# facebookresearch/multipathnet

Hardware: NVIDIA H100
Metric: proposals/sec (higher is better)
Workload: dtype fp32 (wgmma split emulation, fp32 accumulate: 3 bf16 products per MAC, 2 fp16 products in fc6/fc7)

## Files before the change

### multipathnet_b200/csrc/gemm_tc.cu

```cuda
#include "conv_gemm.cuh"
#include "wgmma.cuh"
#include "fp8_e4m3.cuh"
#include <algorithm>
#include <stdlib.h>
#include <string.h>

namespace {

constexpr int BM = 128;
constexpr int BK = 64;
constexpr int TC_THREADS = 384;
constexpr int CONS_THREADS = 256;
constexpr int A_TILE_BYTES = BM * BK * 2;
constexpr int SMEM_BUDGET = 196608;

__host__ __device__ constexpr int a_planes(OperandScheme ops) { return (ops == OperandScheme::BF16X1 || ops == OperandScheme::FP8X1) ? 1 : 2; }
__host__ __device__ constexpr int b_planes(OperandScheme ops) { return ops == OperandScheme::BF16X3 ? 2 : 1; }
__host__ __device__ constexpr int elem_bytes(OperandScheme ops) { return ops == OperandScheme::FP8X1 ? 1 : 2; }
__host__ __device__ constexpr int a_tile_bytes(OperandScheme ops) { return BM * BK * elem_bytes(ops); }
__host__ __device__ constexpr int stage_bytes(int BN, OperandScheme ops = OperandScheme::BF16X3) {
  return a_planes(ops) * a_tile_bytes(ops) + b_planes(ops) * BN * BK * elem_bytes(ops);
}
__host__ __device__ constexpr int max_stages(OperandScheme ops) { return ops == OperandScheme::FP8X1 ? 8 : 4; }
__host__ __device__ constexpr int num_stages(int BN, OperandScheme ops = OperandScheme::BF16X3) {
  return (SMEM_BUDGET / stage_bytes(BN, ops)) > max_stages(ops) ? max_stages(ops) : (SMEM_BUDGET / stage_bytes(BN, ops));
}
__host__ __device__ constexpr int stg_ld(int BN) { return BN + 4; }
static_assert(BM * (256 + 4) * 4 <= 2 * stage_bytes(256), "staging tile must fit in the ring");

struct TcParams {
  int N, Ho, Wo, Cout;
  int kh, kw, stride, pad;
  int cblocks;
  int tn, th, tw;
  int tiles_img, tiles_h, tiles_w, tiles_n;
  const float *bias;
  const __nv_bfloat16 *res_hi, *res_lo; long long res_ld;
  __nv_bfloat16 *out_hi, *out_lo; long long out_ld;
  float *out_f32; long long out_f32_ld;
  __nv_bfloat16 *pool_hi, *pool_lo; long long pool_ld; int Hp, Wp;
  int relu;
  int splitk, kb_per_split;
  long long split_stride;
  unsigned long long *tl_min, *tl_max;
  float acc_scale;
  int out_fmt;
  unsigned *ovf;
  const int *a_exp, *b_exp; long long sample_pix;
};

__device__ __forceinline__ unsigned long long gtimer() {
  unsigned long long t; asm volatile("mov.u64 %0, %%globaltimer;" : "=l"(t)); return t;
}
__device__ __forceinline__ void tl_min_stamp(const unsigned long long *base_, int i) {
  if (base_) atomicMin(const_cast<unsigned long long *>(base_) + i, gtimer());
}
__device__ __forceinline__ void tl_max_stamp(const unsigned long long *base_, int i) {
  if (base_) atomicMax(const_cast<unsigned long long *>(base_) + i, gtimer());
}
__device__ __forceinline__ uint32_t smem_u32(const void *p) { return (uint32_t)__cvta_generic_to_shared(p); }
__device__ __forceinline__ void mbar_init(uint32_t bar, uint32_t count) {
  asm volatile("mbarrier.init.shared::cta.b64 [%0], %1;" ::"r"(bar), "r"(count) : "memory");
}
__device__ __forceinline__ void mbar_expect_tx(uint32_t bar, uint32_t bytes) {
  asm volatile("mbarrier.arrive.expect_tx.shared::cta.b64 _, [%0], %1;" ::"r"(bar), "r"(bytes) : "memory");
}
__device__ __forceinline__ void mbar_arrive(uint32_t bar) {
  asm volatile("mbarrier.arrive.shared::cta.b64 _, [%0];" ::"r"(bar) : "memory");
}
__device__ __forceinline__ void mbar_wait(uint32_t bar, uint32_t parity) {
  uint32_t done;
  uint32_t spins = 0;
  do {
    asm volatile(
        "{\n\t.reg .pred p;\n\t"
        "mbarrier.try_wait.parity.shared::cta.b64 p, [%1], %2;\n\t"
        "selp.u32 %0, 1, 0, p;\n\t}"
        : "=r"(done) : "r"(bar), "r"(parity) : "memory");
    if (!done && ++spins == (1u << 26)) __trap();
  } while (!done);
}
__device__ __forceinline__ void tma_load_4d(uint32_t dst, const CUtensorMap *tm, uint32_t bar, int c0, int c1,
                                            int c2, int c3) {
  asm volatile(
      "cp.async.bulk.tensor.4d.shared::cluster.global.mbarrier::complete_tx::bytes [%0], [%1, {%3, %4, %5, %6}], [%2];"
      ::"r"(dst), "l"(reinterpret_cast<uint64_t>(tm)), "r"(bar), "r"(c0), "r"(c1), "r"(c2), "r"(c3) : "memory");
}
__device__ __forceinline__ void tma_load_2d(uint32_t dst, const CUtensorMap *tm, uint32_t bar, int c0, int c1) {
  asm volatile(
      "cp.async.bulk.tensor.2d.shared::cluster.global.mbarrier::complete_tx::bytes [%0], [%1, {%3, %4}], [%2];"
      ::"r"(dst), "l"(reinterpret_cast<uint64_t>(tm)), "r"(bar), "r"(c0), "r"(c1) : "memory");
}
__device__ __forceinline__ void prefetch_tmap(const CUtensorMap *tm) {
  asm volatile("prefetch.tensormap [%0];" ::"l"(reinterpret_cast<uint64_t>(tm)) : "memory");
}
__device__ __forceinline__ void consumers_sync() { asm volatile("bar.sync 1, 256;" ::: "memory"); }

__device__ __forceinline__ uint64_t make_smem_desc(uint32_t saddr) {
  uint64_t d = 0;
  d |= (uint64_t)((saddr & 0x3FFFFu) >> 4);
  d |= (uint64_t)1 << 16;
  d |= (uint64_t)(1024 >> 4) << 32;
  d |= (uint64_t)1 << 62;
  return d;
}

__device__ __forceinline__ uint64_t make_smem_desc_64b(uint32_t saddr) {
  uint64_t d = 0;
  d |= (uint64_t)((saddr & 0x3FFFFu) >> 4);
  d |= (uint64_t)1 << 16;
  d |= (uint64_t)(512 >> 4) << 32;
  d |= (uint64_t)2 << 62;
  return d;
}

template <int BN, OperandScheme OPS>
__device__ __forceinline__ void mma_kblock(float (&acc)[BN / 2], uint64_t a_hi, uint64_t a_lo, uint64_t b_hi, uint64_t b_lo, bool first) {
  constexpr bool F16 = (OPS == OperandScheme::FP16X2);
#pragma unroll
  for (int k = 0; k < BK / 16; ++k) {
    const uint64_t adv = (uint64_t)((k * 16 * 2) >> 4);
    const uint32_t later = (first && k == 0) ? 0u : 1u;
    if constexpr (OPS == OperandScheme::BF16X1) {
      wgmma_nk16<BN, false>(acc, a_hi + adv, b_hi + adv, later);
    } else {
      wgmma_nk16<BN, F16>(acc, a_lo + adv, b_hi + adv, later);
      if (!F16) wgmma_nk16<BN, F16>(acc, a_hi + adv, b_lo + adv, 1u);
      wgmma_nk16<BN, F16>(acc, a_hi + adv, b_hi + adv, 1u);
    }
  }
}

template <int BN>
__device__ __forceinline__ void stage_acc(float *stg, const float (&acc)[BN / 2], int g, int t) {
  const int r0 = g * 64 + (t >> 5) * 16 + ((t & 31) >> 2), c0 = 2 * (t & 3);
#pragma unroll
  for (int j = 0; j < BN / 8; ++j) {
    *reinterpret_cast<float2 *>(stg + r0 * stg_ld(BN) + 8 * j + c0) = make_float2(acc[4 * j], acc[4 * j + 1]);
    *reinterpret_cast<float2 *>(stg + (r0 + 8) * stg_ld(BN) + 8 * j + c0) = make_float2(acc[4 * j + 2], acc[4 * j + 3]);
  }
}

template <int BN, OperandScheme OPS>
__device__ __forceinline__ void epilogue_row(const TcParams &p, const float *srow, int nt, bool row_ok, long long pix,
                                             float *out_f32, int ch_first, long long ppix) {
  const bool pool = (p.pool_hi != nullptr);
  const int tile_end = min(p.Cout, nt * BN + BN);
#pragma unroll 1
  for (int ch = ch_first; ch < BN / 32; ch += 2) {
    const int col0 = nt * BN + ch * 32;
    if (col0 >= tile_end) break;
    float v[32];
#pragma unroll
    for (int j = 0; j < 8; ++j) {
      const float4 x = *reinterpret_cast<const float4 *>(srow + ch * 32 + 4 * j);
      v[4 * j] = x.x; v[4 * j + 1] = x.y; v[4 * j + 2] = x.z; v[4 * j + 3] = x.w;
    }
    if (OPS == OperandScheme::FP16X2) {
#pragma unroll
      for (int e = 0; e < 32; ++e) v[e] *= p.acc_scale;
    }
    if (OPS == OperandScheme::FP8X1) {
      const int ea = row_ok ? __ldg(p.a_exp + pix / p.sample_pix) : 0;
#pragma unroll
      for (int e = 0; e < 32; ++e) v[e] *= mpn_fp8::pow2(-(ea + __ldg(p.b_exp + col0 + e)));
    }
    if (!(row_ok || pool)) continue;
#pragma unroll
    for (int g = 0; g < 4; ++g) {
      const int c = col0 + g * 8;
      if (c >= tile_end) break;
      float f[8];
#pragma unroll
      for (int e = 0; e < 8; ++e) f[e] = v[g * 8 + e];
      const bool full8 = (c + 8 <= tile_end);
      if (p.bias) {
        if (full8) {
          const float4 b0 = __ldg(reinterpret_cast<const float4 *>(p.bias + c));
          const float4 b1 = __ldg(reinterpret_cast<const float4 *>(p.bias + c + 4));
          f[0] += b0.x; f[1] += b0.y; f[2] += b0.z; f[3] += b0.w;
          f[4] += b1.x; f[5] += b1.y; f[6] += b1.z; f[7] += b1.w;
        } else {
          for (int e = 0; e < 8 && c + e < p.Cout; ++e) f[e] += __ldg(p.bias + c + e);
        }
      }
      if (p.res_hi && full8 && row_ok) {
        const uint4 rh = *reinterpret_cast<const uint4 *>(p.res_hi + pix * p.res_ld + c);
        const uint4 rl = *reinterpret_cast<const uint4 *>(p.res_lo + pix * p.res_ld + c);
        const uint32_t hh[4] = {rh.x, rh.y, rh.z, rh.w}, ll[4] = {rl.x, rl.y, rl.z, rl.w};
#pragma unroll
        for (int t = 0; t < 4; ++t) {
          float2 x = bf16x2_to_float2(hh[t]), y = bf16x2_to_float2(ll[t]);
          f[2 * t] += x.x + y.x; f[2 * t + 1] += x.y + y.y;
        }
      }
      if (p.relu) {
#pragma unroll
        for (int e = 0; e < 8; ++e) f[e] = fmaxf(f[e], 0.f);
      }
      if (p.out_hi && full8 && row_ok) {
        uint32_t oh[4], ol[4];
#pragma unroll
        for (int t = 0; t < 4; ++t) split_x2(p.out_fmt, f[2 * t], f[2 * t + 1], oh[t], ol[t], p.ovf);
        *reinterpret_cast<uint4 *>(p.out_hi + pix * p.out_ld + c) = make_uint4(oh[0], oh[1], oh[2], oh[3]);
        *reinterpret_cast<uint4 *>(p.out_lo + pix * p.out_ld + c) = make_uint4(ol[0], ol[1], ol[2], ol[3]);
      }
      if (pool) {
#pragma unroll
        for (int e = 0; e < 8; ++e) {
          float x = row_ok ? f[e] : -INFINITY;
          x = fmaxf(x, __shfl_xor_sync(0xffffffffu, x, 1));
          x = fmaxf(x, __shfl_xor_sync(0xffffffffu, x, 8));
          f[e] = x;
        }
        if (ppix >= 0 && full8) {
          uint32_t oh[4], ol[4];
#pragma unroll
          for (int t = 0; t < 4; ++t) split_x2(p.out_fmt, f[2 * t], f[2 * t + 1], oh[t], ol[t], p.ovf);
          *reinterpret_cast<uint4 *>(p.pool_hi + ppix * p.pool_ld + c) = make_uint4(oh[0], oh[1], oh[2], oh[3]);
          *reinterpret_cast<uint4 *>(p.pool_lo + ppix * p.pool_ld + c) = make_uint4(ol[0], ol[1], ol[2], ol[3]);
        }
      }
      if (out_f32 && row_ok) {
        float *o = out_f32 + pix * p.out_f32_ld + c;
        if (full8 && ((reinterpret_cast<uintptr_t>(o) & 15) == 0)) {
          reinterpret_cast<float4 *>(o)[0] = make_float4(f[0], f[1], f[2], f[3]);
          reinterpret_cast<float4 *>(o)[1] = make_float4(f[4], f[5], f[6], f[7]);
        } else {
          for (int e = 0; e < 8 && c + e < p.Cout; ++e) o[e] = f[e];
        }
      }
    }
  }
}

template <int BN, OperandScheme OPS = OperandScheme::BF16X3>
__global__ void __launch_bounds__(TC_THREADS, 1)
conv_gemm_tc_kernel(const __grid_constant__ CUtensorMap tmA_hi, const __grid_constant__ CUtensorMap tmA_lo,
                    const __grid_constant__ CUtensorMap tmB_hi, const __grid_constant__ CUtensorMap tmB_lo,
                    const TcParams p) {
  constexpr int S = num_stages(BN, OPS);
  constexpr int STAGE = stage_bytes(BN, OPS);
  constexpr int A_TILE = a_tile_bytes(OPS);
  constexpr int B_TILE_BYTES = BN * BK * elem_bytes(OPS);
  constexpr int B_OFF = a_planes(OPS) * A_TILE;
  static_assert(BM * stg_ld(BN) * 4 <= S * STAGE, "staging tile must fit in the ring");
  extern __shared__ uint8_t smem_raw[];
  uint8_t *smem = reinterpret_cast<uint8_t *>((reinterpret_cast<uintptr_t>(smem_raw) + 1023) & ~(uintptr_t)1023);
  uint64_t *bars = reinterpret_cast<uint64_t *>(smem + (size_t)S * STAGE);
  const uint32_t smem_base = smem_u32(smem);
  const uint32_t bar_base = smem_u32(bars);
  auto full_bar = [&](int s) { return bar_base + 8u * s; };
  auto empty_bar = [&](int s) { return bar_base + 8u * (S + s); };

  const int tid = threadIdx.x, lane = tid & 31;
  const int unit = (int)blockIdx.x;
  const int tile = unit / p.splitk, split = unit - tile * p.splitk;
  const int nt = tile % p.tiles_n, mt = tile / p.tiles_n;
  const int twi = mt % p.tiles_w, thi = (mt / p.tiles_w) % p.tiles_h, tni = mt / (p.tiles_w * p.tiles_h);
  const int num_kb = p.kh * p.kw * p.cblocks;
  const int kb0 = split * p.kb_per_split, kb1 = min(num_kb, kb0 + p.kb_per_split);

  if (tid == 0) {
    tl_min_stamp(p.tl_min, 0);
    if (a_planes(OPS) == 1) { prefetch_tmap(&tmA_hi); prefetch_tmap(&tmB_hi); }
    else { prefetch_tmap(&tmA_hi); prefetch_tmap(&tmA_lo); prefetch_tmap(&tmB_hi); prefetch_tmap(&tmB_lo); }
    for (int s = 0; s < S; ++s) { mbar_init(full_bar(s), 1); mbar_init(empty_bar(s), CONS_THREADS / 32); }
    asm volatile("fence.mbarrier_init.release.cluster;" ::: "memory");
  }
  __syncthreads();
  asm volatile("griddepcontrol.wait;" ::: "memory");
  asm volatile("griddepcontrol.launch_dependents;" ::: "memory");
  if (tid == 0) tl_min_stamp(p.tl_min, 1);

  if (tid < 128) {
    if (tid == 0) {
      const int w_in0 = twi * p.tw * p.stride - p.pad, h_in0 = thi * p.th * p.stride - p.pad, n0 = tni * p.tn;
      const int b_row0 = nt * BN;
      for (int kb = kb0, it = 0; kb < kb1; ++kb, ++it) {
        const int s = it % S; const uint32_t ph = (uint32_t)(it / S) & 1u;
        mbar_wait(empty_bar(s), ph ^ 1u);
        const int tap = kb / p.cblocks, cb = kb - tap * p.cblocks;
        const int khi = tap / p.kw, kwi = tap - khi * p.kw;
        const uint32_t sa = smem_base + (uint32_t)s * STAGE;
        mbar_expect_tx(full_bar(s), (uint32_t)STAGE);
        tma_load_4d(sa, &tmA_hi, full_bar(s), cb * BK, w_in0 + kwi, h_in0 + khi, n0);
        if (a_planes(OPS) == 2) tma_load_4d(sa + A_TILE, &tmA_lo, full_bar(s), cb * BK, w_in0 + kwi, h_in0 + khi, n0);
        tma_load_2d(sa + B_OFF, &tmB_hi, full_bar(s), kb * BK, b_row0);
        if (b_planes(OPS) == 2) tma_load_2d(sa + B_OFF + B_TILE_BYTES, &tmB_lo, full_bar(s), kb * BK, b_row0);
      }
    }
    return;
  }

  const int e = tid - 128;
  const int g = e >> 7, t = e & 127;
  float acc[BN / 2];
#pragma unroll
  for (int i = 0; i < BN / 2; ++i) acc[i] = 0.f;
  if constexpr (OPS == OperandScheme::FP8X1) {
    float part[BN / 2];
#pragma unroll
    for (int i = 0; i < BN / 2; ++i) part[i] = 0.f;
    for (int kb = kb0, it = 0; kb < kb1; ++kb, ++it) {
      const int s = it % S; const uint32_t ph = (uint32_t)(it / S) & 1u;
      mbar_wait(full_bar(s), ph);
      if (it == 0 && e == 0) tl_min_stamp(p.tl_min, 2);
      const uint32_t sa = smem_base + (uint32_t)s * STAGE;
      const uint64_t a8 = make_smem_desc_64b(sa + (uint32_t)g * (A_TILE / 2));
      const uint64_t b8 = make_smem_desc_64b(sa + B_OFF);
#pragma unroll
      for (int k = 0; k < BK / 32; ++k) {
        wgmma_fence_acc(part);
        wgmma_fence();
        wgmma_e4m3_nk32<BN>(part, a8 + (uint64_t)(2 * k), b8 + (uint64_t)(2 * k), 0u);
        wgmma_commit();
        wgmma_wait<0>();
        wgmma_fence_acc(part);
#pragma unroll
        for (int i = 0; i < BN / 2; ++i) acc[i] += part[i];
      }
      if (lane == 0) mbar_arrive(empty_bar(s));
    }
  } else {
  for (int kb = kb0, it = 0; kb < kb1; ++kb, ++it) {
    const int s = it % S; const uint32_t ph = (uint32_t)(it / S) & 1u;
    mbar_wait(full_bar(s), ph);
    if (it == 0 && e == 0) tl_min_stamp(p.tl_min, 2);
    const uint32_t sa = smem_base + (uint32_t)s * STAGE;
    const uint64_t a_hi = make_smem_desc(sa + (uint32_t)g * (A_TILE / 2));
    const uint64_t a_lo = make_smem_desc(sa + A_TILE + (uint32_t)g * (A_TILE / 2));
    const uint64_t b_hi = make_smem_desc(sa + B_OFF);
    const uint64_t b_lo = make_smem_desc(sa + B_OFF + B_TILE_BYTES);
    wgmma_fence_acc(acc);
    wgmma_fence();
    mma_kblock<BN, OPS>(acc, a_hi, a_lo, b_hi, b_lo, it == 0);
    wgmma_commit();
    wgmma_wait<1>();
    wgmma_fence_acc(acc);
    if (it > 0 && lane == 0) mbar_arrive(empty_bar((it - 1) % S));
  }
  wgmma_wait<0>();
  wgmma_fence_acc(acc);
  }
  if (e == 0) tl_max_stamp(p.tl_max, 0);
  consumers_sync();
  float *stg = reinterpret_cast<float *>(smem);
  stage_acc<BN>(stg, acc, g, t);
  consumers_sync();

  const int row = e & 127;
  const int wl = row & (p.tw - 1), hl = (row / p.tw) & (p.th - 1), nl = row / (p.tw * p.th);
  const int wo = twi * p.tw + wl, ho = thi * p.th + hl, n = tni * p.tn + nl;
  const bool row_ok = (wo < p.Wo) && (ho < p.Ho) && (n < p.N);
  const long long pix = ((long long)n * p.Ho + ho) * p.Wo + wo;
  const long long ppix = (p.pool_hi && row_ok && !(lane & 9)) ? ((long long)n * p.Hp + (ho >> 1)) * p.Wp + (wo >> 1) : -1;
  float *const out_f32 = p.out_f32 ? p.out_f32 + (long long)split * p.split_stride : nullptr;
  epilogue_row<BN, OPS>(p, stg + row * stg_ld(BN), nt, row_ok, pix, out_f32, e >> 7, ppix);
  if (e == 0) tl_max_stamp(p.tl_max, 1);
}

constexpr int C1_THREADS = 256;
constexpr int C1_A_BYTES = 2 * A_TILE_BYTES;
constexpr int C1_B_BYTES = 2 * 64 * 128;
constexpr int C1_OUT_WARP = 16 * 128;
constexpr int C1_SMEM = 2 * C1_A_BYTES + C1_B_BYTES + (C1_THREADS / 32) * C1_OUT_WARP + 1024;

__device__ __forceinline__ void conv1_gather(const float *__restrict__ x, int pix, int pixels, int H, int W, int bhalf,
                                             float (&in)[16]) {
#pragma unroll
  for (int k = 0; k < 16; ++k) in[k] = 0.f;
  if (pix < pixels) {
    const int HW = H * W;
    const int n = pix / HW, rem = pix - n * HW;
    const int ho = rem / W, wo = rem - ho * W;
    const float *x0 = x + ((size_t)n * 3 * HW + (size_t)(ho - 1) * W + (wo - 1));
    const bool rok[3] = {ho >= 1, true, ho + 1 < H}, cok[3] = {wo >= 1, true, wo + 1 < W};
#pragma unroll
    for (int k = 0; k < 16; ++k) {
      const int kk = 16 * bhalf + k;
      if (kk < 27) {
        const int ci = kk / 9, r = (kk / 3) % 3, q = kk % 3;
        in[k] = (rok[r] && cok[q]) ? __ldg(x0 + ci * HW + r * W + q) : 0.f;
      }
    }
  }
}

__device__ __forceinline__ void conv1_store_plane(uint32_t so, const uint32_t (&v)[16], __nv_bfloat16 *out, int pix0,
                                                  int pixels, int lane) {
  const int r = lane >> 2;
  const uint32_t wr = so + (uint32_t)(r * 128 + 4 * (lane & 3));
  __syncwarp();
#pragma unroll
  for (int j = 0; j < 8; ++j) {
    const uint32_t a = wr + (uint32_t)((j ^ r) * 16);
    asm volatile("st.shared.b32 [%0], %1;" ::"r"(a), "r"(v[j]) : "memory");
    asm volatile("st.shared.b32 [%0], %1;" ::"r"(a + 8 * 128), "r"(v[8 + j]) : "memory");
  }
  __syncwarp();
  const int row0 = lane >> 3, ch = lane & 7;
  const uint32_t rd0 = so + (uint32_t)(row0 * 128 + ((ch ^ row0) * 16)), rd1 = so + (uint32_t)(row0 * 128 + ((ch ^ row0 ^ 4) * 16));
  __nv_bfloat16 *o = out + (size_t)(pix0 + row0) * 64 + ch * 8;
#pragma unroll
  for (int q = 0; q < 4; ++q) {
    uint4 d;
    asm volatile("ld.shared.v4.b32 {%0, %1, %2, %3}, [%4];" : "=r"(d.x), "=r"(d.y), "=r"(d.z), "=r"(d.w)
                 : "r"(((q & 1) ? rd1 : rd0) + (uint32_t)(q * 4 * 128)) : "memory");
    if (pix0 + row0 + 4 * q < pixels) *reinterpret_cast<uint4 *>(o + q * 4 * 64) = d;
  }
}

__global__ void __launch_bounds__(C1_THREADS, 2)
conv1_tc_kernel(const float *__restrict__ x, int N, int H, int W, const float *__restrict__ w, const float *__restrict__ bias,
                int relu, __nv_bfloat16 *__restrict__ out_hi, __nv_bfloat16 *__restrict__ out_lo) {
  extern __shared__ uint8_t smem_raw[];
  uint8_t *smem = reinterpret_cast<uint8_t *>((reinterpret_cast<uintptr_t>(smem_raw) + 1023) & ~(uintptr_t)1023);
  uint8_t *sB = smem + 2 * C1_A_BYTES;
  const int tid = threadIdx.x, lane = tid & 31, warp = tid >> 5;
  const uint32_t so = smem_u32(sB + C1_B_BYTES) + (uint32_t)(warp * C1_OUT_WARP);
  const uint32_t b_base = smem_u32(sB);
  const int g = tid >> 7;
  const int pixels = N * H * W;
  const int total_tiles = (pixels + BM - 1) / BM;
  asm volatile("griddepcontrol.wait;" ::: "memory");
  asm volatile("griddepcontrol.launch_dependents;" ::: "memory");
  const int c0 = 2 * (lane & 3);
  for (int i = tid; i < 64 * 4; i += C1_THREADS) {
    const int row = i >> 2, j = i & 3;
    uint32_t hh[4], ll[4];
#pragma unroll
    for (int q = 0; q < 4; ++q) {
      const int k0 = j * 8 + 2 * q;
      const float v0 = (k0 < 27) ? __ldg(w + row * 27 + k0) : 0.f, v1 = (k0 + 1 < 27) ? __ldg(w + row * 27 + k0 + 1) : 0.f;
      split_bf16x2(v0, v1, hh[q], ll[q]);
    }
    const uint32_t off = (uint32_t)row * 128u + (uint32_t)((j ^ (row & 7)) * 16);
    *reinterpret_cast<uint4 *>(sB + off) = make_uint4(hh[0], hh[1], hh[2], hh[3]);
    *reinterpret_cast<uint4 *>(sB + 64 * 128 + off) = make_uint4(ll[0], ll[1], ll[2], ll[3]);
  }
  const int brow = tid & 127, bhalf = tid >> 7;
  float in[16];
  conv1_gather(x, (int)blockIdx.x * BM + brow, pixels, H, W, bhalf, in);
  for (int tile = blockIdx.x, it = 0; tile < total_tiles; tile += gridDim.x, ++it) {
    uint8_t *sa = smem + (it & 1) * C1_A_BYTES;
    uint8_t *pa = sa + (size_t)brow * 128;
#pragma unroll
    for (int jj = 0; jj < 2; ++jj) {
      const int j = 2 * bhalf + jj;
      uint32_t hh[4], ll[4];
#pragma unroll
      for (int q = 0; q < 4; ++q) split_bf16x2(in[jj * 8 + 2 * q], in[jj * 8 + 2 * q + 1], hh[q], ll[q]);
      const int pj = (j ^ (brow & 7)) * 16;
      *reinterpret_cast<uint4 *>(pa + pj) = make_uint4(hh[0], hh[1], hh[2], hh[3]);
      *reinterpret_cast<uint4 *>(pa + A_TILE_BYTES + pj) = make_uint4(ll[0], ll[1], ll[2], ll[3]);
    }
    asm volatile("fence.proxy.async.shared::cta;" ::: "memory");
    __syncthreads();
    float acc[32];
#pragma unroll
    for (int i = 0; i < 32; ++i) acc[i] = 0.f;
    const uint32_t a_base = smem_u32(sa);
    const uint64_t a_hi = make_smem_desc(a_base + (uint32_t)g * (A_TILE_BYTES / 2));
    const uint64_t a_lo = make_smem_desc(a_base + A_TILE_BYTES + (uint32_t)g * (A_TILE_BYTES / 2));
    const uint64_t b_hi = make_smem_desc(b_base), b_lo = make_smem_desc(b_base + 64 * 128);
    wgmma_fence_acc(acc);
    wgmma_fence();
#pragma unroll
    for (int k = 0; k < 2; ++k) {
      const uint64_t adv = (uint64_t)((k * 16 * 2) >> 4);
      wgmma_nk16<64, false>(acc, a_lo + adv, b_hi + adv, k ? 1u : 0u);
      wgmma_nk16<64, false>(acc, a_hi + adv, b_lo + adv, 1u);
      wgmma_nk16<64, false>(acc, a_hi + adv, b_hi + adv, 1u);
    }
    wgmma_commit();
    const int next = tile + (int)gridDim.x;
    conv1_gather(x, next < total_tiles ? next * BM + brow : pixels, pixels, H, W, bhalf, in);
    wgmma_wait<0>();
    wgmma_fence_acc(acc);
#pragma unroll
    for (int j = 0; j < 8; ++j) {
      const float2 b = __ldg(reinterpret_cast<const float2 *>(bias + 8 * j + c0));
#pragma unroll
      for (int h = 0; h < 2; ++h) {
        float &f0 = acc[4 * j + 2 * h], &f1 = acc[4 * j + 2 * h + 1];
        f0 += b.x; f1 += b.y;
        if (relu) { f0 = fmaxf(f0, 0.f); f1 = fmaxf(f1, 0.f); }
      }
    }
    const int pix0 = tile * BM + 64 * g + 16 * (warp & 3);
#pragma unroll 1
    for (int plane = 0; plane < 2; ++plane) {
      uint32_t v[16];
#pragma unroll
      for (int j = 0; j < 8; ++j)
#pragma unroll
        for (int h = 0; h < 2; ++h) {
          uint32_t hi2, lo2;
          split_bf16x2(acc[4 * j + 2 * h], acc[4 * j + 2 * h + 1], hi2, lo2);
          v[8 * h + j] = plane ? lo2 : hi2;
        }
      conv1_store_plane(so, v, plane ? out_lo : out_hi, pix0, pixels, lane);
    }
  }
}

struct ReduceParams {
  const float *ws; long long split_stride; int splitk; long long pixels; int Cout;
  const float *bias; const __nv_bfloat16 *res_hi, *res_lo; long long res_ld; int relu;
  __nv_bfloat16 *out_hi, *out_lo; long long out_ld; float *out_f32; long long out_f32_ld;
  OutScatter scatter;
};
__global__ void __launch_bounds__(256) splitk_reduce_kernel(const ReduceParams r) {
  MPN_PDL_SYNC();
  const long long idx = (long long)blockIdx.x * blockDim.x + threadIdx.x;
  if (idx >= r.pixels * r.Cout) return;
  const long long pix = idx / r.Cout; const int c = (int)(idx - pix * r.Cout);
  float acc = 0.f;
  for (int s = 0; s < r.splitk; ++s) acc += r.ws[(long long)s * r.split_stride + idx];
  if (r.bias) acc += __ldg(r.bias + c);
  if (r.res_hi) acc += join_bf16(r.res_hi[pix * r.res_ld + c], r.res_lo[pix * r.res_ld + c]);
  if (r.relu) acc = fmaxf(acc, 0.f);
  if (r.out_hi) { __nv_bfloat16 h, l; split_bf16(acc, h, l); r.out_hi[pix * r.out_ld + c] = h; r.out_lo[pix * r.out_ld + c] = l; }
  if (r.scatter.n > 0) {
#pragma unroll 1
    for (int g = 0; g < r.scatter.n; ++g)
      if (c >= r.scatter.seg[g].c0 && c < r.scatter.seg[g].c1) { r.scatter.seg[g].ptr[pix * r.scatter.seg[g].ld + (c - r.scatter.seg[g].c0)] = acc; break; }
  } else if (r.out_f32) r.out_f32[pix * r.out_f32_ld + c] = acc;
}

typedef CUresult (*PFN_encodeTiled)(CUtensorMap *, CUtensorMapDataType, cuuint32_t, void *, const cuuint64_t *,
                                    const cuuint64_t *, const cuuint32_t *, const cuuint32_t *, CUtensorMapInterleave,
                                    CUtensorMapSwizzle, CUtensorMapL2promotion, CUtensorMapFloatOOBfill);
PFN_encodeTiled get_encode_fn() {
  static PFN_encodeTiled fn = nullptr;
  if (!fn) {
    void *p = nullptr; cudaDriverEntryPointQueryResult q;
    if (cudaGetDriverEntryPoint("cuTensorMapEncodeTiled", &p, cudaEnableDefault, &q) == cudaSuccess &&
        q == cudaDriverEntryPointSuccess)
      fn = reinterpret_cast<PFN_encodeTiled>(p);
  }
  return fn;
}

int encode_map(mpn_ctx *ctx, CUtensorMap *tm, const void *base, int rank, const cuuint64_t *dims,
               const cuuint64_t *strides_bytes , const cuuint32_t *box, const cuuint32_t *estr, bool fp8 = false) {
  PFN_encodeTiled fn = get_encode_fn();
  if (!fn) return mpn_fail(ctx, MPN_ERR_CUDA, "cuTensorMapEncodeTiled entry point unavailable");
  CUresult r = fn(tm, fp8 ? CU_TENSOR_MAP_DATA_TYPE_UINT8 : CU_TENSOR_MAP_DATA_TYPE_BFLOAT16, (cuuint32_t)rank, const_cast<void *>(base), dims,
                  strides_bytes, box, estr, CU_TENSOR_MAP_INTERLEAVE_NONE, fp8 ? CU_TENSOR_MAP_SWIZZLE_64B : CU_TENSOR_MAP_SWIZZLE_128B,
                  CU_TENSOR_MAP_L2_PROMOTION_L2_256B, CU_TENSOR_MAP_FLOAT_OOB_FILL_NONE);
  if (r != CUDA_SUCCESS) {
    char b[256];
    snprintf(b, sizeof b, "cuTensorMapEncodeTiled failed (%d): rank %d dims %llu %llu box %u %u", (int)r, rank,
             (unsigned long long)dims[0], (unsigned long long)dims[1], box[0], box[1]);
    return mpn_fail(ctx, MPN_ERR_CUDA, b);
  }
  return MPN_OK;
}

inline bool tc_use_pdl() {
  static const int on = [] { const char *e = getenv("MPN_TC_PDL"); return (e && e[0] == '0') ? 0 : 1; }();
  return on != 0;
}

template <int BN, OperandScheme OPS = OperandScheme::BF16X3>
int launch_bn(mpn_ctx *ctx, const ConvPlan &pl, const TcParams &tp) {
  const int smem = num_stages(BN, OPS) * stage_bytes(BN, OPS) + 1024  + 256 ;
  constexpr int bslot = BN == 256 ? 2 : (BN == 128 ? 1 : 0);
  constexpr int slot = OPS == OperandScheme::FP16X2 ? 3 : (OPS == OperandScheme::BF16X1 ? 5 + bslot
                                                         : (OPS == OperandScheme::FP8X1 ? 8 + bslot : bslot));
  if (!ctx->tc_attr_set[slot]) {
    MPN_CUDA(ctx, cudaFuncSetAttribute(conv_gemm_tc_kernel<BN, OPS>, cudaFuncAttributeMaxDynamicSharedMemorySize, smem));
    ctx->tc_attr_set[slot] = 1;
  }
  const long long units = (long long)pl.tiles_img * pl.tiles_h * pl.tiles_w * pl.tiles_n * pl.splitk;
  MPN_CHECK_ARG(ctx, units > 0 && units < (1ll << 31), "conv_tc: grid size out of range");
  cudaLaunchConfig_t cfg = {};
  cfg.gridDim = dim3((unsigned)units); cfg.blockDim = dim3(TC_THREADS); cfg.dynamicSmemBytes = (size_t)smem; cfg.stream = ctx->stream;
  cudaLaunchAttribute attr[1];
  int na = 0;
  if (tc_use_pdl()) {
    attr[na].id = cudaLaunchAttributeProgrammaticStreamSerialization;
    attr[na].val.programmaticStreamSerializationAllowed = 1;
    ++na;
  }
  cfg.attrs = attr; cfg.numAttrs = na;
  MPN_CUDA(ctx, cudaLaunchKernelEx(&cfg, conv_gemm_tc_kernel<BN, OPS>, pl.tmA_hi, pl.tmA_lo, pl.tmB_hi, pl.tmB_lo, tp));
  MPN_LAUNCHED(ctx);
  return MPN_OK;
}

int launch_ops(mpn_ctx *ctx, const ConvPlan &pl, const TcParams &tp) {
  if (pl.ops == OperandScheme::FP16X2) return launch_bn<256, OperandScheme::FP16X2>(ctx, pl, tp);
  if (pl.ops == OperandScheme::FP8X1)
    return pl.BN == 128 ? launch_bn<128, OperandScheme::FP8X1>(ctx, pl, tp) : launch_bn<64, OperandScheme::FP8X1>(ctx, pl, tp);
  if (pl.ops == OperandScheme::BF16X1) {
    switch (pl.BN) {
      case 256: return launch_bn<256, OperandScheme::BF16X1>(ctx, pl, tp);
      case 128: return launch_bn<128, OperandScheme::BF16X1>(ctx, pl, tp);
      default: return launch_bn<64, OperandScheme::BF16X1>(ctx, pl, tp);
    }
  }
  switch (pl.BN) {
    case 256: return launch_bn<256>(ctx, pl, tp);
    case 128: return launch_bn<128>(ctx, pl, tp);
    default: return launch_bn<64>(ctx, pl, tp);
  }
}

}

int conv1_tc_launch(mpn_ctx *ctx, const float *x_nchw, int N, int H, int W, const float *w_dev, const float *bias_dev, int relu,
                    DTensor &y) {
  MPN_CHECK_ARG(ctx, y.hi && y.lo && y.C == 64 && y.ld % 8 == 0, "conv1_tc: output must be 64-channel split planes");
  MPN_CHECK_ARG(ctx, bias_dev, "conv1_tc: bias missing");
  MPN_CHECK_ARG(ctx, y.ld == 64 && (long long)N * H * W < (1ll << 31) - 256, "conv1_tc: dense 64-channel output and < 2^31 pixels");
  if (!ctx->tc_attr_set[4]) {
    MPN_CUDA(ctx, cudaFuncSetAttribute(conv1_tc_kernel, cudaFuncAttributeMaxDynamicSharedMemorySize, C1_SMEM));
    ctx->tc_attr_set[4] = 1;
  }
  const long long tiles = ((long long)N * H * W + BM - 1) / BM;
  cudaLaunchConfig_t cfg = {};
  cfg.gridDim = dim3((unsigned)std::min<long long>(tiles, 2ll * ctx->sm_count)); cfg.blockDim = dim3(C1_THREADS);
  cfg.dynamicSmemBytes = (size_t)C1_SMEM; cfg.stream = ctx->stream;
  cudaLaunchAttribute attr[1];
  int na = 0;
  if (tc_use_pdl()) { attr[na].id = cudaLaunchAttributeProgrammaticStreamSerialization; attr[na].val.programmaticStreamSerializationAllowed = 1; ++na; }
  cfg.attrs = attr; cfg.numAttrs = na;
  MPN_CUDA(ctx, cudaLaunchKernelEx(&cfg, conv1_tc_kernel, x_nchw, N, H, W, w_dev, bias_dev, relu, y.hi, y.lo));
  MPN_LAUNCHED(ctx);
  return MPN_OK;
}

double conv_flops(const ConvProblem &p) {
  const double Ho = (double)p.y.H, Wo = (double)p.y.W;
  return 2.0 * (double)p.x.C * p.Cout * p.kh * p.kw * Ho * Wo * (double)p.y.N;
}

static int conv_tc_plan_impl(mpn_ctx *ctx, int sm_count, const ConvProblem &p, ConvPlan &pl, bool choose_only) {
  pl.valid = 0;
  MPN_CHECK_ARG(ctx, choose_only || (p.x.hi && p.x.lo && ((p.w_hi && p.w_lo) || p.w16)), "conv_tc: operands must be split-bf16 (or an fp16 weight plane)");
  MPN_CHECK_ARG(ctx, !(p.w16 && p.bf16), "conv_tc: the bf16 numerics do not take an fp16 weight plane");
  MPN_CHECK_ARG(ctx, !(p.fp8 && (p.w16 || p.bf16)), "conv_tc: the fp8 numerics take neither an fp16 weight plane nor the bf16 numerics");
  MPN_CHECK_ARG(ctx, choose_only || !p.fp8 || (p.x8 && p.x8_exp && p.w8 && p.w8_exp), "conv_tc: the fp8 numerics need e4m3 planes and exponents");
  pl.ops = p.w16 ? OperandScheme::FP16X2 : (p.fp8 ? OperandScheme::FP8X1 : (p.bf16 ? OperandScheme::BF16X1 : OperandScheme::BF16X3));
  const bool w16 = pl.ops == OperandScheme::FP16X2, fp8 = pl.ops == OperandScheme::FP8X1;
  MPN_CHECK_ARG(ctx, choose_only || (p.x.fmt == 1) == w16, "conv_tc: fp16 activation planes go with the fp16 weight plane (and only with it)");
  MPN_CHECK_ARG(ctx, p.x.C % BK == 0, "conv_tc: Cin must be a multiple of 64");
  MPN_CHECK_ARG(ctx, p.x.ld % 8 == 0, "conv_tc: input pixel stride must be a multiple of 8 elements");
  MPN_CHECK_ARG(ctx, p.stride >= 1 && p.stride <= 2, "conv_tc: stride must be 1 or 2");
  const int Ho = (int)p.y.H, Wo = (int)p.y.W, N = (int)p.y.N;
  pl.flat = (p.kh == 1 && p.kw == 1 && p.stride == 1 && p.pad == 0) ? 1 : 0;
  pl.mode = 0; pl.splitk = 1;
  cuuint64_t dims[4], strides[3]; cuuint32_t box[4], estr[4];
  int gtn = 1, gth = 1, gtw = BM;
  if (!pl.flat) {
    double best = -1.0;
    for (int tw = 1; tw <= 128; tw <<= 1)
      for (int th = 1; th * tw <= 128; th <<= 1) {
        const int tn = 128 / (tw * th);
        if (tw * p.stride > 256 || th * p.stride > 256) continue;
        const long long tiles = (long long)((Wo + tw - 1) / tw) * ((Ho + th - 1) / th) * ((N + tn - 1) / tn);
        const double util = (double)N * Ho * Wo / (double)(tiles * 128) + 1e-6 * tw;
        if (util > best) { best = util; gtn = tn; gth = th; gtw = tw; }
      }
  }
  const long long P = (long long)p.x.N * p.x.H * p.x.W;
  {
    const bool r3_ok = (p.kh == 3 && p.kw == 3 && p.stride == 1 && p.pad == 1);
    const char *env3 = getenv("MPN_TC_R3");
    const char *env3m = getenv("MPN_TC_R3_MINPIX");
    const long long r3_minpix = env3m ? atoll(env3m) : 0;
    pl.mode = (r3_ok && !(env3 && env3[0] == '0') && P >= r3_minpix) ? 1 : 0;
  }
  const long long tiles_m = pl.flat ? (P + BM - 1) / BM
                                    : (pl.mode ? (long long)((Wo + 7) / 8) * ((Ho + 15) / 16) * N
                                               : (long long)((Wo + gtw - 1) / gtw) * ((Ho + gth - 1) / gth) * ((N + gtn - 1) / gtn));
  {
    const int taps = p.kh * p.kw;
    const double kblocks = (double)taps * (double)(p.x.C / BK);
    double best = 1e300; int best_bn = 64;
    for (int bi = 0; bi < 3; ++bi) {
      const int bn = bi == 0 ? 256 : (bi == 1 ? 128 : 64);
      if (w16 && bn != 256) continue;
      if (fp8 && bn == 256) continue;
      if (!p.m_invariant && bn > 64 && bn > ((p.Cout + 63) / 64) * 64) continue;
      const int roi_bn = p.Cout > 128 ? 256 : (p.Cout > 64 ? 128 : 64);
      if (p.m_invariant && bn != (fp8 ? std::min(roi_bn, 128) : roi_bn)) continue;
      const long long units = tiles_m * ((p.Cout + bn - 1) / bn);
      const long long rounds = (units + sm_count - 1) / sm_count;
      const double mma = (w16 ? 2.0 : (pl.ops == OperandScheme::BF16X1 ? 1.0 : (fp8 ? 0.5 : 3.0))) * 128.0 * bn * 64.0 / 1024.0;
      const double ingest = ((double)a_planes(pl.ops) * 128 + (double)b_planes(pl.ops) * bn) * (fp8 ? 64.0 : 128.0) / 48.0;
      const double cost = (double)rounds * (kblocks * std::max(mma, ingest) + 1500.0 + 8.0 * bn);
      if (cost < best * 0.999) { best = cost; best_bn = bn; }
    }
    pl.BN = best_bn;
    pl.tiles_n = (p.Cout + pl.BN - 1) / pl.BN;
  }
  if (pl.flat) {
    pl.tn = 1; pl.th = 1; pl.tw = BM;
    pl.tiles_img = 1; pl.tiles_h = 1; pl.tiles_w = (int)((P + BM - 1) / BM);
    dims[0] = (cuuint64_t)p.x.C; dims[1] = (cuuint64_t)P; dims[2] = 1; dims[3] = 1;
    strides[0] = (cuuint64_t)p.x.ld * 2; strides[1] = (cuuint64_t)P * p.x.ld * 2; strides[2] = strides[1];
    box[0] = BK; box[1] = BM; box[2] = 1; box[3] = 1;
    estr[0] = estr[1] = estr[2] = estr[3] = 1;
  } else {
    if (pl.mode == 1) { pl.tn = 1; pl.th = 16; pl.tw = 8; }
    else { pl.tn = gtn; pl.th = gth; pl.tw = gtw; }
    pl.tiles_w = (Wo + pl.tw - 1) / pl.tw; pl.tiles_h = (Ho + pl.th - 1) / pl.th; pl.tiles_img = (N + pl.tn - 1) / pl.tn;
    dims[0] = (cuuint64_t)p.x.C; dims[1] = (cuuint64_t)p.x.W; dims[2] = (cuuint64_t)p.x.H; dims[3] = (cuuint64_t)p.x.N;
    strides[0] = (cuuint64_t)p.x.ld * 2; strides[1] = (cuuint64_t)p.x.W * p.x.ld * 2;
    strides[2] = (cuuint64_t)p.x.H * p.x.W * p.x.ld * 2;
    box[0] = BK; box[1] = (cuuint32_t)(pl.tw * p.stride); box[2] = (cuuint32_t)(pl.th * p.stride); box[3] = (cuuint32_t)pl.tn;
    estr[0] = 1; estr[1] = (cuuint32_t)p.stride; estr[2] = (cuuint32_t)p.stride; estr[3] = 1;
  }
  {
    const long long units = tiles_m * pl.tiles_n;
    const long long num_kb = (long long)p.kh * p.kw * (p.x.C / BK);
    long long sk = std::min<long long>(num_kb / 8, 8);
    if (p.m_invariant) { if (!(pl.flat && p.Cout <= 128) || sk < 2) sk = 1; }
    else if (pl.mode == 1 || sk < 2 || units * sk > sm_count) sk = 1;
    const char *env2 = getenv("MPN_TC_SPLITK");
    if (env2 && env2[0] == '0') sk = 1;
    pl.splitk = (int)std::max<long long>(sk, 1);
    pl.kb_per_split = (int)((num_kb + pl.splitk - 1) / pl.splitk);
    pl.splitk = (int)((num_kb + pl.kb_per_split - 1) / pl.kb_per_split);
  }
  if (choose_only) return MPN_OK;
  const long long Ktot = (long long)p.kh * p.kw * p.x.C;
  cuuint64_t bd[2] = {(cuuint64_t)Ktot, (cuuint64_t)p.Cout}, bs[1] = {(cuuint64_t)Ktot * 2};
  cuuint32_t bb[2] = {BK, (cuuint32_t)pl.BN}, be[2] = {1, 1};
  if (fp8) {
    const cuuint64_t C8 = (cuuint64_t)p.x.C;
    if (pl.flat) { strides[0] = C8; strides[1] = (cuuint64_t)P * C8; strides[2] = strides[1]; }
    else { strides[0] = C8; strides[1] = (cuuint64_t)p.x.W * C8; strides[2] = (cuuint64_t)p.x.H * p.x.W * C8; }
    bs[0] = (cuuint64_t)Ktot;
    MPN_TRY(encode_map(ctx, &pl.tmA_hi, p.x8, 4, dims, strides, box, estr, true));
    MPN_TRY(encode_map(ctx, &pl.tmB_hi, p.w8, 2, bd, bs, bb, be, true));
    pl.tmA_lo = pl.tmA_hi; pl.tmB_lo = pl.tmB_hi;
    pl.valid = 1;
    return MPN_OK;
  }
  MPN_TRY(encode_map(ctx, &pl.tmA_hi, p.x.hi, 4, dims, strides, box, estr));
  if (a_planes(pl.ops) == 2) { MPN_TRY(encode_map(ctx, &pl.tmA_lo, p.x.lo, 4, dims, strides, box, estr)); }
  else pl.tmA_lo = pl.tmA_hi;
  if (w16) {
    MPN_CHECK_ARG(ctx, pl.mode == 0 && pl.flat && pl.splitk == 1 && pl.BN == 256, "conv_tc: the fp16-weight path is for wide flat GEMMs without split-K");
    MPN_TRY(encode_map(ctx, &pl.tmB_hi, p.w16, 2, bd, bs, bb, be));
    pl.tmB_lo = pl.tmB_hi;
  } else {
    MPN_TRY(encode_map(ctx, &pl.tmB_hi, p.w_hi, 2, bd, bs, bb, be));
    if (b_planes(pl.ops) == 2) { MPN_TRY(encode_map(ctx, &pl.tmB_lo, p.w_lo, 2, bd, bs, bb, be)); }
    else pl.tmB_lo = pl.tmB_hi;
  }
  pl.valid = 1;
  return MPN_OK;
}

int conv_tc_plan(mpn_ctx *ctx, const ConvProblem &p, ConvPlan &pl) { return conv_tc_plan_impl(ctx, ctx->sm_count, p, pl, false); }

int conv_tc_launch(mpn_ctx *ctx, const ConvProblem &p, const ConvPlan &pl) {
  MpnProfScope prof_scope__(ctx, MPN_CAT_CONV_TC);
  MPN_CHECK_ARG(ctx, pl.valid, "conv_tc_launch: invalid plan");
  TcParams tp;
  memset(&tp, 0, sizeof(tp));
  if (pl.flat) { tp.N = 1; tp.Ho = 1; tp.Wo = (int)(p.y.N * p.y.H * p.y.W); }
  else { tp.N = (int)p.y.N; tp.Ho = (int)p.y.H; tp.Wo = (int)p.y.W; }
  tp.Cout = p.Cout; tp.kh = p.kh; tp.kw = p.kw; tp.stride = p.stride; tp.pad = p.pad;
  tp.cblocks = (int)(p.x.C / BK);
  tp.tn = pl.tn; tp.th = pl.th; tp.tw = pl.tw;
  tp.tiles_img = pl.tiles_img; tp.tiles_h = pl.tiles_h; tp.tiles_w = pl.tiles_w; tp.tiles_n = pl.tiles_n;
  tp.bias = p.bias;
  tp.res_hi = p.res.hi; tp.res_lo = p.res.lo; tp.res_ld = p.res.ld;
  tp.out_hi = p.y.hi; tp.out_lo = p.y.lo; tp.out_ld = p.y.ld;
  tp.out_f32 = p.y.f32; tp.out_f32_ld = p.y_f32_ld;
  tp.relu = p.relu;
  tp.splitk = pl.splitk; tp.kb_per_split = pl.kb_per_split; tp.split_stride = 0;
  tp.acc_scale = pl.ops == OperandScheme::FP16X2 ? p.w16_inv_scale : 1.f;
  tp.out_fmt = p.y.fmt; tp.ovf = nullptr;
  if (p.y.fmt) MPN_TRY(mpn_ovf_flag(ctx, &tp.ovf));
  if (pl.ops == OperandScheme::FP8X1) { tp.a_exp = p.x8_exp; tp.b_exp = p.w8_exp; tp.sample_pix = p.y.H * p.y.W; }
  MPN_CHECK_ARG(ctx, !p.pool.hi || p.pool.fmt == p.y.fmt, "conv_tc: pooled output must share the output's plane format");
  MPN_CHECK_ARG(ctx, !(p.y.fmt && pl.splitk > 1), "conv_tc: fp16 output planes are not written by the split-K reduce");
  MPN_CHECK_ARG(ctx, !p.res.hi || p.res.fmt == 0, "conv_tc: residual inputs are bf16 split planes");
  if (ctx->tl_on && ctx->tl_n < ctx->tl_cap) { tp.tl_min = ctx->tl_min + 4 * ctx->tl_n; tp.tl_max = ctx->tl_max + 4 * ctx->tl_n; ++ctx->tl_n; }
  if (p.pool.hi) {
    MPN_CHECK_ARG(ctx, pl.mode == 1 && pl.splitk == 1 && !p.res.hi && p.Cout % 8 == 0 && p.pool.ld % 8 == 0,
                  "conv_tc: fused pooling needs the 3x3 kernel, no residual, Cout multiple of 8");
    MPN_CHECK_ARG(ctx, p.pool.H == (p.y.H + 1) / 2 && p.pool.W == (p.y.W + 1) / 2 && p.pool.N == p.y.N, "conv_tc: pooled geometry mismatch");
    tp.pool_hi = p.pool.hi; tp.pool_lo = p.pool.lo; tp.pool_ld = p.pool.ld; tp.Hp = (int)p.pool.H; tp.Wp = (int)p.pool.W;
    if (p.pool_only) { tp.out_hi = tp.out_lo = nullptr; tp.out_f32 = nullptr; }
  }
  if (p.y.hi) MPN_CHECK_ARG(ctx, p.Cout % 8 == 0 && p.y.ld % 8 == 0, "conv_tc: split output needs Cout, ld multiples of 8");
  MPN_CHECK_ARG(ctx, p.scatter.n == 0 || pl.splitk > 1, "conv_tc: scattered outputs need a split-K plan");
  if (pl.splitk > 1) {
    const long long pixels = (long long)p.y.N * p.y.H * p.y.W;
    float *ws = nullptr;
    MPN_TRY(mpn_scratch3(ctx, sizeof(float) * (size_t)pl.splitk * pixels * p.Cout, (void **)&ws));
    tp.bias = nullptr; tp.res_hi = tp.res_lo = nullptr; tp.relu = 0; tp.out_hi = tp.out_lo = nullptr;
    tp.out_f32 = ws; tp.out_f32_ld = p.Cout; tp.split_stride = pixels * p.Cout;
    MPN_TRY(launch_ops(ctx, pl, tp));
    ReduceParams r;
    r.ws = ws; r.split_stride = tp.split_stride; r.splitk = pl.splitk; r.pixels = pixels; r.Cout = p.Cout;
    r.bias = p.bias; r.res_hi = p.res.hi; r.res_lo = p.res.lo; r.res_ld = p.res.ld; r.relu = p.relu;
    r.out_hi = p.y.hi; r.out_lo = p.y.lo; r.out_ld = p.y.ld; r.out_f32 = p.y.f32; r.out_f32_ld = p.y_f32_ld;
    r.scatter = p.scatter;
    const long long total = pixels * p.Cout;
    MPN_CUDA(ctx, mpn_launch_pdl(ctx, splitk_reduce_kernel, dim3((unsigned)((total + 255) / 256)), dim3(256), 0, r));
    MPN_LAUNCHED(ctx);
    return MPN_OK;
  }
  return launch_ops(ctx, pl, tp);
}

extern "C" int mpn_debug_plan(int64_t N, int64_t Cin, int64_t H, int64_t W, int64_t Cout, int32_t k, int32_t stride, int32_t pad,
                              int32_t per_roi, int32_t sm_count, int32_t *out) {
  if (!out || N <= 0 || Cin <= 0 || Cin % 64 || H <= 0 || W <= 0 || Cout <= 0 || k <= 0 || stride < 1 || stride > 2 || pad < 0 || sm_count < 2)
    return MPN_ERR_ARG;
  ConvProblem p;
  p.x.N = N; p.x.H = H; p.x.W = W; p.x.C = Cin; p.x.ld = Cin;
  p.Cout = (int)Cout; p.kh = p.kw = k; p.stride = stride; p.pad = pad; p.m_invariant = per_roi ? 1 : 0;
  p.y.N = N; p.y.H = (H + 2 * pad - k) / stride + 1; p.y.W = (W + 2 * pad - k) / stride + 1; p.y.C = Cout; p.y.ld = Cout;
  if (p.y.H <= 0 || p.y.W <= 0) return MPN_ERR_ARG;
  ConvPlan pl;
  const int rc = conv_tc_plan_impl(nullptr, sm_count, p, pl, true);
  if (rc != MPN_OK) return rc;
  out[0] = pl.mode; out[1] = 1; out[2] = pl.BN; out[3] = pl.splitk; out[4] = 0; out[5] = pl.tn; out[6] = pl.th; out[7] = pl.tw;
  return MPN_OK;
}
```

Before: 292,800.

## Split K-blocks into half-depth stages with 64B swizzle for BN=256 tiles

For BN=256 tiles, each 64-wide K block is now split into two 32-element stages using 64-byte swizzled TMA boxes and matching wgmma descriptors. This halves the bytes per stage and allows up to 8 ring stages instead of the 2 that fit before. The aim is a deeper producer/consumer pipeline that hides TMA latency better for wide tiles. The cost is twice as many mbarrier waits and commits per K block, plus smaller TMA transactions.

```diff
diff --git a/multipathnet_b200/csrc/gemm_tc.cu b/multipathnet_b200/csrc/gemm_tc.cu
--- a/multipathnet_b200/csrc/gemm_tc.cu
+++ b/multipathnet_b200/csrc/gemm_tc.cu
@@ -17,16 +17,21 @@
 __host__ __device__ constexpr int a_planes(OperandScheme ops) { return (ops == OperandScheme::BF16X1 || ops == OperandScheme::FP8X1) ? 1 : 2; }
 __host__ __device__ constexpr int b_planes(OperandScheme ops) { return ops == OperandScheme::BF16X3 ? 2 : 1; }
 __host__ __device__ constexpr int elem_bytes(OperandScheme ops) { return ops == OperandScheme::FP8X1 ? 1 : 2; }
-__host__ __device__ constexpr int a_tile_bytes(OperandScheme ops) { return BM * BK * elem_bytes(ops); }
+__host__ __device__ constexpr int row_bytes(int BN, OperandScheme ops) { return (ops == OperandScheme::FP8X1 || BN == 256) ? 64 : 128; }
+__host__ __device__ constexpr int stage_k(int BN, OperandScheme ops) { return row_bytes(BN, ops) / elem_bytes(ops); }
+__host__ __device__ constexpr int kb_steps(int BN, OperandScheme ops) { return BK / stage_k(BN, ops); }
+__host__ __device__ constexpr int a_tile_bytes(int BN, OperandScheme ops) { return BM * row_bytes(BN, ops); }
 __host__ __device__ constexpr int stage_bytes(int BN, OperandScheme ops = OperandScheme::BF16X3) {
-  return a_planes(ops) * a_tile_bytes(ops) + b_planes(ops) * BN * BK * elem_bytes(ops);
-}
-__host__ __device__ constexpr int max_stages(OperandScheme ops) { return ops == OperandScheme::FP8X1 ? 8 : 4; }
+  return (a_planes(ops) * BM + b_planes(ops) * BN) * row_bytes(BN, ops);
+}
+__host__ __device__ constexpr int max_stages(int BN, OperandScheme ops) { return row_bytes(BN, ops) == 64 ? 8 : 4; }
 __host__ __device__ constexpr int num_stages(int BN, OperandScheme ops = OperandScheme::BF16X3) {
-  return (SMEM_BUDGET / stage_bytes(BN, ops)) > max_stages(ops) ? max_stages(ops) : (SMEM_BUDGET / stage_bytes(BN, ops));
+  return (SMEM_BUDGET / stage_bytes(BN, ops)) > max_stages(BN, ops) ? max_stages(BN, ops) : (SMEM_BUDGET / stage_bytes(BN, ops));
+}
+__host__ __device__ constexpr int tc_smem_bytes(int BN, OperandScheme ops) {
+  return num_stages(BN, ops) * stage_bytes(BN, ops) + 1024  + 256 ;
 }
 __host__ __device__ constexpr int stg_ld(int BN) { return BN + 4; }
-static_assert(BM * (256 + 4) * 4 <= 2 * stage_bytes(256), "staging tile must fit in the ring");
 
 struct TcParams {
   int N, Ho, Wo, Cout;
@@ -115,10 +120,10 @@
 }
 
 template <int BN, OperandScheme OPS>
-__device__ __forceinline__ void mma_kblock(float (&acc)[BN / 2], uint64_t a_hi, uint64_t a_lo, uint64_t b_hi, uint64_t b_lo, bool first) {
+__device__ __forceinline__ void mma_kstep(float (&acc)[BN / 2], uint64_t a_hi, uint64_t a_lo, uint64_t b_hi, uint64_t b_lo, bool first) {
   constexpr bool F16 = (OPS == OperandScheme::FP16X2);
 #pragma unroll
-  for (int k = 0; k < BK / 16; ++k) {
+  for (int k = 0; k < stage_k(BN, OPS) / 16; ++k) {
     const uint64_t adv = (uint64_t)((k * 16 * 2) >> 4);
     const uint32_t later = (first && k == 0) ? 0u : 1u;
     if constexpr (OPS == OperandScheme::BF16X1) {
@@ -241,10 +246,12 @@
                     const TcParams p) {
   constexpr int S = num_stages(BN, OPS);
   constexpr int STAGE = stage_bytes(BN, OPS);
-  constexpr int A_TILE = a_tile_bytes(OPS);
-  constexpr int B_TILE_BYTES = BN * BK * elem_bytes(OPS);
+  constexpr int A_TILE = a_tile_bytes(BN, OPS);
+  constexpr int B_TILE_BYTES = BN * row_bytes(BN, OPS);
   constexpr int B_OFF = a_planes(OPS) * A_TILE;
+  constexpr int KSTEPS = kb_steps(BN, OPS);
   static_assert(BM * stg_ld(BN) * 4 <= S * STAGE, "staging tile must fit in the ring");
+  static_assert(S >= 2 && 2 * S * 8 <= 256, "ring depth: at least two stages, barriers in their 256 bytes");
   extern __shared__ uint8_t smem_raw[];
   uint8_t *smem = reinterpret_cast<uint8_t *>((reinterpret_cast<uintptr_t>(smem_raw) + 1023) & ~(uintptr_t)1023);
   uint64_t *bars = reinterpret_cast<uint64_t *>(smem + (size_t)S * STAGE);
@@ -277,17 +284,21 @@
     if (tid == 0) {
       const int w_in0 = twi * p.tw * p.stride - p.pad, h_in0 = thi * p.th * p.stride - p.pad, n0 = tni * p.tn;
       const int b_row0 = nt * BN;
-      for (int kb = kb0, it = 0; kb < kb1; ++kb, ++it) {
-        const int s = it % S; const uint32_t ph = (uint32_t)(it / S) & 1u;
-        mbar_wait(empty_bar(s), ph ^ 1u);
+      for (int kb = kb0, it = 0; kb < kb1; ++kb) {
         const int tap = kb / p.cblocks, cb = kb - tap * p.cblocks;
         const int khi = tap / p.kw, kwi = tap - khi * p.kw;
-        const uint32_t sa = smem_base + (uint32_t)s * STAGE;
-        mbar_expect_tx(full_bar(s), (uint32_t)STAGE);
-        tma_load_4d(sa, &tmA_hi, full_bar(s), cb * BK, w_in0 + kwi, h_in0 + khi, n0);
-        if (a_planes(OPS) == 2) tma_load_4d(sa + A_TILE, &tmA_lo, full_bar(s), cb * BK, w_in0 + kwi, h_in0 + khi, n0);
-        tma_load_2d(sa + B_OFF, &tmB_hi, full_bar(s), kb * BK, b_row0);
-        if (b_planes(OPS) == 2) tma_load_2d(sa + B_OFF + B_TILE_BYTES, &tmB_lo, full_bar(s), kb * BK, b_row0);
+#pragma unroll
+        for (int h = 0; h < KSTEPS; ++h, ++it) {
+          const int s = it % S; const uint32_t ph = (uint32_t)(it / S) & 1u;
+          const int ka = cb * BK + h * stage_k(BN, OPS), kk = kb * BK + h * stage_k(BN, OPS);
+          mbar_wait(empty_bar(s), ph ^ 1u);
+          const uint32_t sa = smem_base + (uint32_t)s * STAGE;
+          mbar_expect_tx(full_bar(s), (uint32_t)STAGE);
+          tma_load_4d(sa, &tmA_hi, full_bar(s), ka, w_in0 + kwi, h_in0 + khi, n0);
+          if (a_planes(OPS) == 2) tma_load_4d(sa + A_TILE, &tmA_lo, full_bar(s), ka, w_in0 + kwi, h_in0 + khi, n0);
+          tma_load_2d(sa + B_OFF, &tmB_hi, full_bar(s), kk, b_row0);
+          if (b_planes(OPS) == 2) tma_load_2d(sa + B_OFF + B_TILE_BYTES, &tmB_lo, full_bar(s), kk, b_row0);
+        }
       }
     }
     return;
@@ -323,18 +334,20 @@
       if (lane == 0) mbar_arrive(empty_bar(s));
     }
   } else {
-  for (int kb = kb0, it = 0; kb < kb1; ++kb, ++it) {
+  const int steps = (kb1 - kb0) * KSTEPS;
+  for (int it = 0; it < steps; ++it) {
     const int s = it % S; const uint32_t ph = (uint32_t)(it / S) & 1u;
     mbar_wait(full_bar(s), ph);
     if (it == 0 && e == 0) tl_min_stamp(p.tl_min, 2);
     const uint32_t sa = smem_base + (uint32_t)s * STAGE;
-    const uint64_t a_hi = make_smem_desc(sa + (uint32_t)g * (A_TILE / 2));
-    const uint64_t a_lo = make_smem_desc(sa + A_TILE + (uint32_t)g * (A_TILE / 2));
-    const uint64_t b_hi = make_smem_desc(sa + B_OFF);
-    const uint64_t b_lo = make_smem_desc(sa + B_OFF + B_TILE_BYTES);
+    auto desc = [](uint32_t a) { return row_bytes(BN, OPS) == 64 ? make_smem_desc_64b(a) : make_smem_desc(a); };
+    const uint64_t a_hi = desc(sa + (uint32_t)g * (A_TILE / 2));
+    const uint64_t a_lo = desc(sa + A_TILE + (uint32_t)g * (A_TILE / 2));
+    const uint64_t b_hi = desc(sa + B_OFF);
+    const uint64_t b_lo = desc(sa + B_OFF + B_TILE_BYTES);
     wgmma_fence_acc(acc);
     wgmma_fence();
-    mma_kblock<BN, OPS>(acc, a_hi, a_lo, b_hi, b_lo, it == 0);
+    mma_kstep<BN, OPS>(acc, a_hi, a_lo, b_hi, b_lo, it == 0);
     wgmma_commit();
     wgmma_wait<1>();
     wgmma_fence_acc(acc);
@@ -544,11 +557,12 @@
 }
 
 int encode_map(mpn_ctx *ctx, CUtensorMap *tm, const void *base, int rank, const cuuint64_t *dims,
-               const cuuint64_t *strides_bytes , const cuuint32_t *box, const cuuint32_t *estr, bool fp8 = false) {
+               const cuuint64_t *strides_bytes , const cuuint32_t *box, const cuuint32_t *estr, int BN, OperandScheme ops) {
+  const bool fp8 = ops == OperandScheme::FP8X1;
   PFN_encodeTiled fn = get_encode_fn();
   if (!fn) return mpn_fail(ctx, MPN_ERR_CUDA, "cuTensorMapEncodeTiled entry point unavailable");
   CUresult r = fn(tm, fp8 ? CU_TENSOR_MAP_DATA_TYPE_UINT8 : CU_TENSOR_MAP_DATA_TYPE_BFLOAT16, (cuuint32_t)rank, const_cast<void *>(base), dims,
-                  strides_bytes, box, estr, CU_TENSOR_MAP_INTERLEAVE_NONE, fp8 ? CU_TENSOR_MAP_SWIZZLE_64B : CU_TENSOR_MAP_SWIZZLE_128B,
+                  strides_bytes, box, estr, CU_TENSOR_MAP_INTERLEAVE_NONE, row_bytes(BN, ops) == 64 ? CU_TENSOR_MAP_SWIZZLE_64B : CU_TENSOR_MAP_SWIZZLE_128B,
                   CU_TENSOR_MAP_L2_PROMOTION_L2_256B, CU_TENSOR_MAP_FLOAT_OOB_FILL_NONE);
   if (r != CUDA_SUCCESS) {
     char b[256];
@@ -566,7 +580,7 @@
 
 template <int BN, OperandScheme OPS = OperandScheme::BF16X3>
 int launch_bn(mpn_ctx *ctx, const ConvPlan &pl, const TcParams &tp) {
-  const int smem = num_stages(BN, OPS) * stage_bytes(BN, OPS) + 1024  + 256 ;
+  const int smem = tc_smem_bytes(BN, OPS);
   constexpr int bslot = BN == 256 ? 2 : (BN == 128 ? 1 : 0);
   constexpr int slot = OPS == OperandScheme::FP16X2 ? 3 : (OPS == OperandScheme::BF16X1 ? 5 + bslot
                                                          : (OPS == OperandScheme::FP8X1 ? 8 + bslot : bslot));
@@ -703,7 +717,7 @@
     pl.tiles_img = 1; pl.tiles_h = 1; pl.tiles_w = (int)((P + BM - 1) / BM);
     dims[0] = (cuuint64_t)p.x.C; dims[1] = (cuuint64_t)P; dims[2] = 1; dims[3] = 1;
     strides[0] = (cuuint64_t)p.x.ld * 2; strides[1] = (cuuint64_t)P * p.x.ld * 2; strides[2] = strides[1];
-    box[0] = BK; box[1] = BM; box[2] = 1; box[3] = 1;
+    box[0] = (cuuint32_t)stage_k(pl.BN, pl.ops); box[1] = BM; box[2] = 1; box[3] = 1;
     estr[0] = estr[1] = estr[2] = estr[3] = 1;
   } else {
     if (pl.mode == 1) { pl.tn = 1; pl.th = 16; pl.tw = 8; }
@@ -712,7 +726,7 @@
     dims[0] = (cuuint64_t)p.x.C; dims[1] = (cuuint64_t)p.x.W; dims[2] = (cuuint64_t)p.x.H; dims[3] = (cuuint64_t)p.x.N;
     strides[0] = (cuuint64_t)p.x.ld * 2; strides[1] = (cuuint64_t)p.x.W * p.x.ld * 2;
     strides[2] = (cuuint64_t)p.x.H * p.x.W * p.x.ld * 2;
-    box[0] = BK; box[1] = (cuuint32_t)(pl.tw * p.stride); box[2] = (cuuint32_t)(pl.th * p.stride); box[3] = (cuuint32_t)pl.tn;
+    box[0] = (cuuint32_t)stage_k(pl.BN, pl.ops); box[1] = (cuuint32_t)(pl.tw * p.stride); box[2] = (cuuint32_t)(pl.th * p.stride); box[3] = (cuuint32_t)pl.tn;
     estr[0] = 1; estr[1] = (cuuint32_t)p.stride; estr[2] = (cuuint32_t)p.stride; estr[3] = 1;
   }
   {
@@ -730,28 +744,28 @@
   if (choose_only) return MPN_OK;
   const long long Ktot = (long long)p.kh * p.kw * p.x.C;
   cuuint64_t bd[2] = {(cuuint64_t)Ktot, (cuuint64_t)p.Cout}, bs[1] = {(cuuint64_t)Ktot * 2};
-  cuuint32_t bb[2] = {BK, (cuuint32_t)pl.BN}, be[2] = {1, 1};
+  cuuint32_t bb[2] = {(cuuint32_t)stage_k(pl.BN, pl.ops), (cuuint32_t)pl.BN}, be[2] = {1, 1};
   if (fp8) {
     const cuuint64_t C8 = (cuuint64_t)p.x.C;
     if (pl.flat) { strides[0] = C8; strides[1] = (cuuint64_t)P * C8; strides[2] = strides[1]; }
     else { strides[0] = C8; strides[1] = (cuuint64_t)p.x.W * C8; strides[2] = (cuuint64_t)p.x.H * p.x.W * C8; }
     bs[0] = (cuuint64_t)Ktot;
-    MPN_TRY(encode_map(ctx, &pl.tmA_hi, p.x8, 4, dims, strides, box, estr, true));
-    MPN_TRY(encode_map(ctx, &pl.tmB_hi, p.w8, 2, bd, bs, bb, be, true));
+    MPN_TRY(encode_map(ctx, &pl.tmA_hi, p.x8, 4, dims, strides, box, estr, pl.BN, pl.ops));
+    MPN_TRY(encode_map(ctx, &pl.tmB_hi, p.w8, 2, bd, bs, bb, be, pl.BN, pl.ops));
     pl.tmA_lo = pl.tmA_hi; pl.tmB_lo = pl.tmB_hi;
     pl.valid = 1;
     return MPN_OK;
   }
-  MPN_TRY(encode_map(ctx, &pl.tmA_hi, p.x.hi, 4, dims, strides, box, estr));
-  if (a_planes(pl.ops) == 2) { MPN_TRY(encode_map(ctx, &pl.tmA_lo, p.x.lo, 4, dims, strides, box, estr)); }
+  MPN_TRY(encode_map(ctx, &pl.tmA_hi, p.x.hi, 4, dims, strides, box, estr, pl.BN, pl.ops));
+  if (a_planes(pl.ops) == 2) { MPN_TRY(encode_map(ctx, &pl.tmA_lo, p.x.lo, 4, dims, strides, box, estr, pl.BN, pl.ops)); }
   else pl.tmA_lo = pl.tmA_hi;
   if (w16) {
     MPN_CHECK_ARG(ctx, pl.mode == 0 && pl.flat && pl.splitk == 1 && pl.BN == 256, "conv_tc: the fp16-weight path is for wide flat GEMMs without split-K");
-    MPN_TRY(encode_map(ctx, &pl.tmB_hi, p.w16, 2, bd, bs, bb, be));
+    MPN_TRY(encode_map(ctx, &pl.tmB_hi, p.w16, 2, bd, bs, bb, be, pl.BN, pl.ops));
     pl.tmB_lo = pl.tmB_hi;
   } else {
-    MPN_TRY(encode_map(ctx, &pl.tmB_hi, p.w_hi, 2, bd, bs, bb, be));
-    if (b_planes(pl.ops) == 2) { MPN_TRY(encode_map(ctx, &pl.tmB_lo, p.w_lo, 2, bd, bs, bb, be)); }
+    MPN_TRY(encode_map(ctx, &pl.tmB_hi, p.w_hi, 2, bd, bs, bb, be, pl.BN, pl.ops));
+    if (b_planes(pl.ops) == 2) { MPN_TRY(encode_map(ctx, &pl.tmB_lo, p.w_lo, 2, bd, bs, bb, be, pl.BN, pl.ops)); }
     else pl.tmB_lo = pl.tmB_hi;
   }
   pl.valid = 1;
```

Result: faster. 320,500 (median of 6 runs) (+9.5%).
